# mdejong/MetalBT709Decoder

Measured on AMD Instinct MI355X. Metric: Gpixel/s, 4k NV12->sRGB BGRA decode (output pixels), higher is better.
Workload: dtype f32

## Files before the change

include/bt709hip_ext.h:

```cpp
#ifndef BT709HIP_EXT_H
#define BT709HIP_EXT_H

#include "bt709hip.h"

#ifdef __cplusplus
extern "C" {
#endif

typedef struct bt709hip_pool bt709hip_pool;

typedef struct {
  int32_t device_ordinal;
  int32_t compute_units;
  int32_t wavefront_size;
  int32_t lds_bytes_per_block;
  int32_t memory_clock_khz;
  int32_t memory_bus_width_bits;
  int32_t l2_bytes;
  int32_t clock_khz;
  uint64_t total_memory_bytes;
  char name[128];
  char arch[64];
  char pci_bus_id[32];
  char uuid[40];
// ... 4 lines not shown
  BT709HIP_CTX_OPT_GRID_MULT = 1,
  BT709HIP_CTX_OPT_ENCODE_ROW_PAIRS = 2,
  BT709HIP_CTX_OPT_ENCODE_THREADS = 3,
  BT709HIP_CTX_OPT_XCD_BANDS = 4,
  BT709HIP_CTX_OPT_STREAMING_TRIES = 5
} bt709hip_context_option;
int bt709hip_context_set_option(bt709hip_context *ctx, int option, int value);

int bt709hip_stream_create_with_priority(bt709hip_context *ctx, int priority, void **stream);

int bt709hip_event_create(bt709hip_context *ctx, void **event);
int bt709hip_event_destroy(bt709hip_context *ctx, void *event);
int bt709hip_event_record(bt709hip_context *ctx, void *event, void *stream);
int bt709hip_event_synchronize(bt709hip_context *ctx, void *event);
int bt709hip_stream_wait_event(bt709hip_context *ctx, void *stream, void *event);
int bt709hip_event_elapsed_ms(bt709hip_context *ctx, void *start, void *stop, float *ms);

int bt709hip_graph_begin_capture(bt709hip_context *ctx, void *stream);
int bt709hip_graph_end_capture(bt709hip_context *ctx, void *stream, void **graph);
int bt709hip_graph_launch(bt709hip_context *ctx, void *graph, void *stream);
int bt709hip_graph_destroy(bt709hip_context *ctx, void *graph);

int bt709hip_mem_info(bt709hip_context *ctx, size_t *free_bytes, size_t *total_bytes);
int bt709hip_host_alloc(bt709hip_context *ctx, size_t bytes, void **hptr);
int bt709hip_host_free(bt709hip_context *ctx, void *hptr);

typedef enum {
  BT709HIP_OPT_NONTEMPORAL = 1,
  BT709HIP_OPT_HALF_KERNEL = 2,
  BT709HIP_OPT_HALF_WORKGROUPS = 3,
  BT709HIP_OPT_HALF_LDS_KB = 4,
  BT709HIP_OPT_XCD_BANDS = 5,
  BT709HIP_OPT_COALESCE = 6,
  BT709HIP_OPT_COALESCE_MAX_AGE_US = 7
} bt709hip_decoder_option;
int bt709hip_decoder_set_option(bt709hip_decoder *dec, int option, int value);
int bt709hip_decoder_get_option(const bt709hip_decoder *dec, int option, int *value);

int bt709hip_decoder_flush(bt709hip_decoder *dec, void *stream );
int bt709hip_decoder_flush_all(bt709hip_decoder *dec);

int bt709hip_unconvert_batch(bt709hip_decoder *dec, int count, const void *const *ycbcr_words, size_t in_stride, int width, int height,
                             const bt709hip_surface *outs, void *stream, int wait_until_completed);
int bt709hip_decode_half_batch(bt709hip_decoder *dec, int count, const bt709hip_frame *frames, const bt709hip_frame *alphas,
                               const bt709hip_surface *outs, void *stream, int wait_until_completed);
int bt709hip_decode_scaled_batch(bt709hip_decoder *dec, int count, const bt709hip_frame *frames, const bt709hip_frame *alphas,
                                 const bt709hip_surface *outs, void *stream, int wait_until_completed);
int bt709hip_render_scaled_batch(bt709hip_context *ctx, int count, const bt709hip_surface *ins, const bt709hip_surface *outs,
                                 void *stream, int wait_until_completed);
int bt709hip_encode_batch(bt709hip_context *ctx, int count, const bt709hip_surface *ins, const bt709hip_frame *outs, int input_gamma,
                          int output_gamma, void *stream, int wait_until_completed);
int bt709hip_render_scaled_prepare(bt709hip_context *ctx);
int bt709hip_decoder_prepare_format(bt709hip_decoder *dec, int format);
int bt709hip_encoder_prepare(bt709hip_context *ctx, int input_gamma, int output_gamma);

int bt709hip_pool_create(bt709hip_decoder *dec, int width, int height, int depth, bt709hip_pool **out);
int bt709hip_pool_destroy(bt709hip_pool *pool);
int bt709hip_pool_acquire(bt709hip_pool *pool, int *slot, void **y, size_t *y_stride, void **cbcr,
                          size_t *cbcr_stride);
int bt709hip_pool_alpha_plane(bt709hip_pool *pool, int slot, void **alpha, size_t *alpha_stride);
int bt709hip_pool_submit(bt709hip_pool *pool, int slot);
int bt709hip_pool_wait(bt709hip_pool *pool, int slot, const void **bgra, size_t *stride);
int bt709hip_pool_release(bt709hip_pool *pool, int slot);

typedef struct bt709hip_ring bt709hip_ring;
typedef struct {
  int32_t tries;
  int32_t in_candidates;
  int32_t out_candidates;
  int32_t chosen_in, chosen_out;
// ... 89 lines not shown
```

metalbt709decoder_amd/_capi.py:

```python
import ctypes as C
import os

from . import build as _build

c_void_pp = C.POINTER(C.c_void_p)


class Frame(C.Structure):
    _fields_ = [("y", C.c_void_p), ("y_stride", C.c_size_t),
                ("cbcr", C.c_void_p), ("cbcr_stride", C.c_size_t),
                ("width", C.c_int32), ("height", C.c_int32),
                ("matrix", C.c_int32), ("transfer", C.c_int32)]


class Surface(C.Structure):
    _fields_ = [("bgra", C.c_void_p), ("stride", C.c_size_t),
                ("width", C.c_int32), ("height", C.c_int32),
                ("format", C.c_int32), ("reserved", C.c_int32)]


ABI_VERSION = 503

FORMAT_BGRA8_SRGB = 0
FORMAT_RGBA16F = 1

OPT_NONTEMPORAL = 1
OPT_HALF_KERNEL = 2
OPT_HALF_WORKGROUPS = 3
OPT_HALF_LDS_KB = 4
OPT_XCD_BANDS = 5
OPT_COALESCE = 6
OPT_COALESCE_MAX_AGE_US = 7
CTX_OPT_GRID_MULT = 1
CTX_OPT_ENCODE_ROW_PAIRS = 2
CTX_OPT_ENCODE_THREADS = 3
CTX_OPT_XCD_BANDS = 4
CTX_OPT_STREAMING_TRIES = 5


class RingPlacement(C.Structure):
    _fields_ = [("tries", C.c_int32), ("in_candidates", C.c_int32), ("out_candidates", C.c_int32),
                ("chosen_in", C.c_int32), ("chosen_out", C.c_int32), ("probes", C.c_int32),
                ("first_GBps", C.c_float), ("chosen_GBps", C.c_float), ("best_GBps", C.c_float), ("worst_GBps", C.c_float),
                ("out_prescan_GBps", C.c_float * 18), ("out_kept", C.c_int32 * 18),
                ("hunt_ms", C.c_float), ("stopped_by", C.c_int32), ("peak_bytes", C.c_uint64), ("budget_bytes", C.c_uint64),
                ("evicted", C.c_int32), ("reserved", C.c_int32)]


class RingOptions(C.Structure):
    _fields_ = [("max_bytes", C.c_uint64), ("max_ms", C.c_uint32), ("frugal", C.c_int32), ("format", C.c_int32), ("reserved", C.c_int32)]


class LaunchInfo(C.Structure):
    _fields_ = [("grid", C.c_uint32 * 3), ("block", C.c_uint32 * 3), ("launches", C.c_int32), ("xcd_bands", C.c_int32)]


class ScaledLaunchInfo(C.Structure):
    _fields_ = [("grid", C.c_uint32 * 3), ("block", C.c_uint32 * 3), ("taps", C.c_uint32), ("rows", C.c_uint32),
                ("persistent", C.c_uint32), ("balanced", C.c_uint32), ("resident", C.c_uint32), ("reserved", C.c_uint32),
                ("items", C.c_uint64)]


SCALED_TAPS_BYTES, SCALED_TAPS_PAIRS, SCALED_TAPS_WIDE, SCALED_TAPS_SHARED, SCALED_TAPS_ONCE = range(5)


# ... 189 lines not shown
```

metalbt709decoder_amd/csrc/bt709_ring.cpp:

```cpp
#include "../../include/bt709hip_ext.h"

#include <algorithm>
#include <chrono>
#include <cstring>
#include <map>
#include <new>
#include <utility>
#include <vector>

struct bt709hip_ring {
  bt709hip_decoder *dec = nullptr;
  bt709hip_context *ctx = nullptr;
  int width = 0, height = 0, frames = 0, half = 0, has_alpha = 0, format = BT709HIP_FORMAT_BGRA8_SRGB;
  size_t y_bytes = 0, c_bytes = 0, in_stride = 0, out_stride = 0;
  void *d_in = nullptr, *d_out = nullptr;
  std::vector<bt709hip_frame> f, a;
  std::vector<bt709hip_surface> o;
  bt709hip_ring_placement placement;
};

namespace {

constexpr size_t kHuntMinBytes = 256u << 20;
constexpr size_t kReserveBytes = 4ull << 30;
// ... 190 lines not shown
  auto time_left = [&]() { return max_s == 0.0 || now_s() - t_start < max_s; };
  pl.tries = tries;
  pl.budget_bytes = led.budget;

  std::vector<Slab> ins, outs;
  {
    int n_in = frugal ? std::min(tries, BT709_HUNT_FRUGAL_INPUTS) : tries;
    while (n_in > 1 && ((!frugal && static_cast<size_t>(n_in) * in_bytes > led.budget / 4) || static_cast<size_t>(n_in) * in_bytes + 2 * out_bytes > led.budget)) --n_in;
    for (int i = 0; i < n_in; ++i) {
      if (i > 0 && !led.fits(in_bytes + out_bytes)) break;
      void *p = led.take(in_bytes);
      if (p == nullptr) break;
      ins.push_back(Slab{p, 0.0f, true});
    }
  }
  auto free_everything = [&]() {
    for (Slab &s : ins)
      if (s.alive) led.give(s.p, in_bytes), s.alive = false;
    for (Slab &s : outs)
      if (s.alive) led.give(s.p, out_bytes), s.alive = false;
  };
  if (!ins.empty()) {
    void *p = led.take(out_bytes);
    if (p != nullptr) outs.push_back(Slab{p, 0.0f, true});
  }
  if (ins.empty() || outs.empty()) {
    free_everything();
    delete r;
    return BT709HIP_ERR_HIP;
  }

  int bi = 0, bo = 0;
  Prober pr{r};
  int coalesce = 0;
  (void)bt709hip_decoder_get_option(dec, BT709HIP_OPT_COALESCE, &coalesce);
  if (tries > 1 && bt709hip_event_create(ctx, &pr.e0) == BT709HIP_OK && bt709hip_event_create(ctx, &pr.e1) == BT709HIP_OK) {
    if (coalesce > 1) (void)bt709hip_decoder_set_option(dec, BT709HIP_OPT_COALESCE, 0);
    const double px_per_launch = static_cast<double>(width) * height * frames;
    pr.bytes_per_launch = (static_cast<double>(r->y_bytes + r->c_bytes + (r->has_alpha ? r->y_bytes : 0)) + static_cast<double>(ow) * oh * static_cast<double>(out_px_bytes)) * frames;
    const int reps = std::max(3, static_cast<int>((8.0 * 256 * 3840 * 2160 + px_per_launch - 1) / px_per_launch));
    auto alive_outs = [&]() { return static_cast<int>(std::count_if(outs.begin(), outs.end(), [](const Slab &s) { return s.alive; })); };
    auto evict_slowest_out = [&]() {
      int worst = -1;
      for (size_t k = 0; k < outs.size(); ++k)
        if (outs[k].alive && (worst < 0 || outs[k].rate < outs[static_cast<size_t>(worst)].rate)) worst = static_cast<int>(k);
      if (worst < 0 || alive_outs() <= 1) return false;
      led.give(outs[static_cast<size_t>(worst)].p, out_bytes);
      outs[static_cast<size_t>(worst)].alive = false;
      ++led.evicted;
      return true;
    };
    outs[0].rate = pr.measure(ins[0].p, outs[0].p, reps, 0.15);
    int target = tries;
    while (pr.rc == BT709HIP_OK) {
      bool stuck = false;
      while (static_cast<int>(outs.size()) < target && pr.rc == BT709HIP_OK) {
        if (!time_left()) {
          pl.stopped_by = 2;
          stuck = true;
          break;
        }
        while (!led.fits(out_bytes) && evict_slowest_out()) pl.stopped_by = pl.stopped_by ? pl.stopped_by : 1;
        void *p = led.fits(out_bytes) ? led.take(out_bytes) : nullptr;
        if (p == nullptr) {
          pl.stopped_by = pl.stopped_by ? pl.stopped_by : 1;
          stuck = true;
          break;
        }
        outs.push_back(Slab{p, 0.0f, true});
        outs.back().rate = pr.measure(ins[0].p, p, reps, BT709_HUNT_WARM_S);
// ... 23 lines not shown
          break;
        }
        probed[{static_cast<int>(i), o}] = i == 0 ? outs[static_cast<size_t>(o)].rate : pr.measure(ins[i].p, outs[static_cast<size_t>(o)].p, reps, BT709_HUNT_WARM_S);
      }
    pl.probes = static_cast<int>(probed.size());
    if (pr.rc == BT709HIP_OK && !probed.empty()) {
      pl.first_GBps = outs[0].rate;
      std::vector<std::pair<float, std::pair<int, int>>> ranked;
      for (const auto &kv : probed) ranked.push_back({kv.second, kv.first});
      std::sort(ranked.begin(), ranked.end(), [](const auto &x, const auto &y) { return x.first > y.first; });
      pl.best_GBps = ranked.front().first;
      pl.worst_GBps = ranked.back().first;
      bi = ranked.front().second.first, bo = ranked.front().second.second;
      pl.chosen_GBps = ranked.front().first;
      std::vector<std::pair<int, int>> finalists;
      for (size_t k = 0; k < ranked.size() && k < 3; ++k) finalists.push_back(ranked[k].second);
      const std::pair<int, int> first_pair{0, 0};
      if (std::find(kept.begin(), kept.end(), 0) != kept.end() && std::find(finalists.begin(), finalists.end(), first_pair) == finalists.end())
        finalists.push_back(first_pair);
      float best = -1.0f;
      if (finalists.size() > 1)
        for (const auto &io : finalists) {
          if (pr.rc != BT709HIP_OK) break;
          if (!time_left()) {
            pl.stopped_by = 2;
            break;
          }
          const float v = pr.measure(ins[static_cast<size_t>(io.first)].p, outs[static_cast<size_t>(io.second)].p, BT709_HUNT_CONFIRM_X * reps, BT709_HUNT_WARM_S);
          if (v > best) best = v, bi = io.first, bo = io.second;
        }
      if (best > 0.0f) pl.chosen_GBps = best;
    }
    if (coalesce > 1) (void)bt709hip_decoder_set_option(dec, BT709HIP_OPT_COALESCE, coalesce);
  }
  if (pr.e0) (void)bt709hip_event_destroy(ctx, pr.e0);
  if (pr.e1) (void)bt709hip_event_destroy(ctx, pr.e1);
  pl.in_candidates = static_cast<int>(ins.size());
  if (pl.out_candidates == 0) pl.out_candidates = static_cast<int>(outs.size());
  pl.chosen_in = bi;
  pl.chosen_out = bo;
  pl.evicted = led.evicted;
  void *keep_in = ins[static_cast<size_t>(bi)].alive ? ins[static_cast<size_t>(bi)].p : nullptr;
  void *keep_out = outs[static_cast<size_t>(bo)].alive ? outs[static_cast<size_t>(bo)].p : nullptr;
  ins[static_cast<size_t>(bi)].alive = false;
  outs[static_cast<size_t>(bo)].alive = false;
  pl.peak_bytes = led.peak;
  free_everything();
  if (pl.tries > 1) pl.hunt_ms = static_cast<float>((now_s() - t_start) * 1e3);
  if (pr.rc != BT709HIP_OK || keep_in == nullptr || keep_out == nullptr) {
    if (keep_in) (void)bt709hip_free(ctx, keep_in);
    if (keep_out) (void)bt709hip_free(ctx, keep_out);
    const int rc = pr.rc != BT709HIP_OK ? pr.rc : BT709HIP_ERR_HIP;
    delete r;
    return rc;
  }
  bind_slabs(r, keep_in, keep_out);
  *out = r;
  return BT709HIP_OK;
}

int bt709hip_ring_frames(const bt709hip_ring *r) { return r ? r->frames : BT709HIP_ERR_INVALID_ARG; }

int bt709hip_ring_frame(const bt709hip_ring *r, int index, bt709hip_frame *frame, bt709hip_frame *alpha, bt709hip_surface *out) {
  if (r == nullptr || index < 0 || index >= r->frames) return BT709HIP_ERR_INVALID_ARG;
  if (frame) *frame = r->f[static_cast<size_t>(index)];
  if (alpha) {
// ... 98 lines not shown
```

metalbt709decoder_amd/csrc/shim_coalesce.cpp:

```cpp
#include "shim_internal.h"

namespace bt709shim __attribute__((visibility("hidden"))) {

int issue_queue(bt709hip_decoder *dec, PendingQueue &q) {
  if (q.frames.empty()) return BT709HIP_OK;
  std::vector<bt709hip_frame> frames, alphas;
  std::vector<bt709hip_surface> outs;
  frames.swap(q.frames);
  alphas.swap(q.alphas);
  outs.swap(q.outs);
  return decode_batch_now(dec, static_cast<int>(frames.size()), frames.data(), q.with_alphas ? alphas.data() : nullptr, outs.data(),
                          q.stream, 0);
}

namespace {
int64_t now_us() {
  return std::chrono::duration_cast<std::chrono::microseconds>(std::chrono::steady_clock::now().time_since_epoch()).count();
}
}

int flush_decoder(bt709hip_decoder *dec, hipStream_t s, bool all, bool aged_only) {
  std::lock_guard<std::mutex> lock(dec->queue_mutex);
  int rc = BT709HIP_OK;
  const int64_t limit = aged_only ? now_us() - dec->coalesce_max_age_us : 0;
  for (PendingQueue &q : dec->queues) {
    if (q.frames.empty()) continue;
    const bool aged = dec->coalesce_max_age_us > 0 && q.oldest_us <= limit;
    if (aged_only ? (aged || q.stream == s) : (all || q.stream == s))
      if (int e = issue_queue(dec, q)) rc = rc ? rc : e;
  }
  return rc;
}

int flush_stream(bt709hip_context *ctx, hipStream_t s, const bt709hip_decoder *skip) {
  if (ctx == nullptr || ctx->n_coalescing.load(std::memory_order_acquire) == 0) return BT709HIP_OK;
  const bool aged_too = !capturing(s);
  std::lock_guard<std::mutex> lock(ctx->coalescing_mutex);
  int rc = BT709HIP_OK;
  for (bt709hip_decoder *d : ctx->coalescing)
    if (d != skip)
      if (int e = flush_decoder(d, s, false, aged_too)) rc = rc ? rc : e;
  return rc;
}

int set_coalescing(bt709hip_decoder *dec, int n) {
  bt709hip_context *ctx = dec->ctx;
  const bool now = n > 1;
  if (now && ctx != nullptr) {
    std::lock_guard<std::mutex> lock(ctx->coalescing_mutex);
    if (std::find(ctx->coalescing.begin(), ctx->coalescing.end(), dec) == ctx->coalescing.end()) ctx->coalescing.push_back(dec);
    ctx->n_coalescing.store(static_cast<int>(ctx->coalescing.size()), std::memory_order_release);
  }
  int rc = BT709HIP_OK;
  {
    std::lock_guard<std::mutex> lock(dec->queue_mutex);
    if (!now)
      for (PendingQueue &q : dec->queues)
        if (int e = issue_queue(dec, q)) rc = rc ? rc : e;
    dec->coalesce.store(now ? n : 0);
  }
  if (!now && ctx != nullptr) {
    std::lock_guard<std::mutex> lock(ctx->coalescing_mutex);
    auto it = std::find(ctx->coalescing.begin(), ctx->coalescing.end(), dec);
    if (it != ctx->coalescing.end()) ctx->coalescing.erase(it);
    ctx->n_coalescing.store(static_cast<int>(ctx->coalescing.size()), std::memory_order_release);
  }
  return rc;
}
// ... 26 lines not shown
    if (q != nullptr)
      if (int rc = issue_queue(dec, *q)) return rc;
    return decode_batch_now(dec, count, frames, alphas, outs, stream, wait_until_completed);
  }
  {
    DecodeParams p;
    BatchInfo info;
    if (int rc = gather_batch(dec, count, frames, alphas, outs, OutShape::kSame, stream, &p, &info)) return rc;
    if (p.width == 0) return BT709HIP_OK;
  }
  if (q == nullptr) {
    dec->queues.emplace_back();
    q = &dec->queues.back();
    q->stream = s;
  }
  if (!q->frames.empty()) {
    const bool fits = q->frames.size() + static_cast<size_t>(count) <= static_cast<size_t>(n) &&
                      same_shape(q->frames[0], frames[0]) && q->frames[0].transfer == frames[0].transfer &&
                      q->outs[0].stride == outs[0].stride && q->outs[0].format == outs[0].format &&
                      q->with_alphas == (alphas != nullptr) && (alphas == nullptr || q->alphas[0].y_stride == alphas[0].y_stride);
    if (!fits)
      if (int rc = issue_queue(dec, *q)) return rc;
  }
  q->with_alphas = alphas != nullptr;
  if (q->frames.empty()) q->oldest_us = now_us();
  q->frames.insert(q->frames.end(), frames, frames + count);
  if (alphas != nullptr) q->alphas.insert(q->alphas.end(), alphas, alphas + count);
  q->outs.insert(q->outs.end(), outs, outs + count);
  set_kernel_name("(queued: coalescing submit)");
  if (q->frames.size() >= static_cast<size_t>(n)) return issue_queue(dec, *q);
  return BT709HIP_OK;
}

}

extern "C" {

int bt709hip_decoder_flush(bt709hip_decoder *dec, void *stream) {
  if (dec == nullptr) return BT709HIP_ERR_INVALID_ARG;
  if (dec->ctx == nullptr) return BT709HIP_OK;
  if (int rc = bind(dec->ctx)) return rc;
  return flush_decoder(dec, pick(dec->ctx, stream), false);
}

int bt709hip_decoder_flush_all(bt709hip_decoder *dec) {
  if (dec == nullptr) return BT709HIP_ERR_INVALID_ARG;
  if (dec->ctx == nullptr) return BT709HIP_OK;
  if (int rc = bind(dec->ctx)) return rc;
  return flush_decoder(dec, nullptr, true);
}

}
```

metalbt709decoder_amd/csrc/shim_core.cpp:

```cpp
#include "shim_internal.h"

namespace bt709shim __attribute__((visibility("hidden"))) {

namespace {
thread_local hipError_t tl_hip_error = hipSuccess;
thread_local const char *tl_kernel_name = "";
thread_local bt709::ScaledLaunchRecord tl_scaled_launch = {};
thread_local bool tl_scaled_launched = false;
}

void set_kernel_name(const char *name) { tl_kernel_name = name; }
const char *kernel_name() { return tl_kernel_name; }
hipError_t last_hip_error() { return tl_hip_error; }
const bt709::ScaledLaunchRecord *scaled_launch() { return tl_scaled_launched ? &tl_scaled_launch : nullptr; }
static void store_scaled_launch(const bt709::ScaledLaunchRecord &record) { tl_scaled_launch = record, tl_scaled_launched = true; }

int hip_fail(hipError_t e) {
  tl_hip_error = e;
  (void)hipGetLastError();
  return BT709HIP_ERR_HIP;
}

int bind(const bt709hip_context *ctx) {
  if (ctx == nullptr) return BT709HIP_ERR_INVALID_ARG;
// ... 68 lines not shown
  *out = ctx;
  return BT709HIP_OK;
}

int bt709hip_abi_version(void) { return BT709HIP_VERSION; }

int bt709hip_context_set_option(bt709hip_context *ctx, int option, int value) {
  if (ctx == nullptr) return BT709HIP_ERR_INVALID_ARG;
  switch (option) {
    case BT709HIP_CTX_OPT_GRID_MULT:
      ctx->grid_mult = value <= 0 ? 2 : clamp_int(value, 1, 64);
      ctx->grid_blocks = ctx->props.multiProcessorCount * 8 * ctx->grid_mult;
      return BT709HIP_OK;
    case BT709HIP_CTX_OPT_ENCODE_ROW_PAIRS:
      ctx->encode_row_pairs = clamp_int(value, 0, 64);
      return BT709HIP_OK;
    case BT709HIP_CTX_OPT_ENCODE_THREADS:
      ctx->encode_threads = clamp_int(value, 0, 1024) / 64 * 64;
      return BT709HIP_OK;
    case BT709HIP_CTX_OPT_XCD_BANDS:
      ctx->xcd_bands = value != 0;
      return BT709HIP_OK;
    case BT709HIP_CTX_OPT_STREAMING_TRIES:
      ctx->streaming_tries = value <= 0 ? 4 : clamp_int(value, 1, 32);
      return BT709HIP_OK;
    default:
      return BT709HIP_ERR_INVALID_ARG;
  }
}

int bt709hip_context_destroy(bt709hip_context *ctx) {
  if (ctx == nullptr) return BT709HIP_OK;
  if (hipSetDevice(ctx->device) == hipSuccess && ctx->default_stream) {
    (void)hipStreamSynchronize(ctx->default_stream);
    (void)hipStreamDestroy(ctx->default_stream);
    for (auto &row : ctx->encoders)
      for (EncoderTables &t : row) {
        if (t.d_per_byte) (void)hipFree(t.d_per_byte);
        if (t.d_from_linear) (void)hipFree(t.d_from_linear);
      }
    if (ctx->d_render_encode) (void)hipFree(ctx->d_render_encode);
    if (ctx->d_render_lin) (void)hipFree(ctx->d_render_lin);
  }
  delete ctx;
  return BT709HIP_OK;
}

int bt709hip_context_info(const bt709hip_context *ctx, bt709hip_device_info *info) {
  if (ctx == nullptr || info == nullptr) return BT709HIP_ERR_INVALID_ARG;
  std::memset(info, 0, sizeof *info);
  info->device_ordinal = ctx->device;
  info->compute_units = ctx->props.multiProcessorCount;
  info->wavefront_size = ctx->props.warpSize;
  info->lds_bytes_per_block = static_cast<int32_t>(ctx->props.sharedMemPerBlock);
  info->memory_clock_khz = ctx->props.memoryClockRate;
  info->memory_bus_width_bits = ctx->props.memoryBusWidth;
  info->l2_bytes = ctx->props.l2CacheSize;
  info->clock_khz = ctx->props.clockRate;
  info->total_memory_bytes = ctx->props.totalGlobalMem;
  std::snprintf(info->name, sizeof info->name, "%s", ctx->props.name);
  std::snprintf(info->arch, sizeof info->arch, "%s", ctx->props.gcnArchName);
  if (hipDeviceGetPCIBusId(info->pci_bus_id, static_cast<int>(sizeof info->pci_bus_id), ctx->device) != hipSuccess) {
    (void)hipGetLastError();
    std::snprintf(info->pci_bus_id, sizeof info->pci_bus_id, "%04x:%02x:%02x.0", ctx->props.pciDomainID, ctx->props.pciBusID, ctx->props.pciDeviceID);
  }
  hipUUID uuid;
// ... 256 lines not shown
```

metalbt709decoder_amd/csrc/shim_decode.cpp:

```cpp
#include "shim_internal.h"

namespace bt709shim __attribute__((visibility("hidden"))) {

int required_transfer(int gamma) {
  switch (gamma) {
    case BT709HIP_GAMMA_SRGB: return BT709HIP_TRANSFER_SRGB;
    case BT709HIP_GAMMA_LINEAR: return BT709HIP_TRANSFER_LINEAR;
    default: return BT709HIP_TRANSFER_ITU_R_709_2;
  }
}

int validate(const bt709hip_decoder *dec, const bt709hip_frame *f, const bt709hip_frame *a,
             const bt709hip_surface *o, int out_w, int out_h, int render_w, int render_h) {
  if (f == nullptr || o == nullptr) return BT709HIP_ERR_INVALID_ARG;
  if (f->width < 0 || f->height < 0) return BT709HIP_ERR_INVALID_ARG;
  if (o->width != out_w || o->height != out_h) return BT709HIP_ERR_SIZE_MISMATCH;
  if (render_w != out_w || render_h != out_h) return BT709HIP_ERR_SIZE_MISMATCH;
  if (a != nullptr && (a->width != f->width || a->height != f->height)) return BT709HIP_ERR_SIZE_MISMATCH;
  if (f->matrix != BT709HIP_MATRIX_ITU_R_709_2) return BT709HIP_ERR_MATRIX;
  if (f->transfer != required_transfer(dec->gamma)) return BT709HIP_ERR_TRANSFER;
  if (a != nullptr && a->transfer != BT709HIP_TRANSFER_LINEAR) return BT709HIP_ERR_ALPHA_TRANSFER;
  if ((f->width & 1) || (f->height & 1)) return BT709HIP_ERR_ODD_DIMENSIONS;
  if (dec->has_alpha && a == nullptr) return BT709HIP_ERR_INVALID_ARG;
  if (f->width == 0 || f->height == 0) return BT709HIP_OK;
// ... 136 lines not shown
  const int n = dec->coalesce;
  (void)set_coalescing(dec, 0);
  dec->ctx = ctx;
  (void)set_coalescing(dec, n);
  return BT709HIP_OK;
}

int bt709hip_decoder_set_alpha_fill(bt709hip_decoder *dec, int alpha_byte) {
  if (dec == nullptr || alpha_byte < 0 || alpha_byte > 255) return BT709HIP_ERR_INVALID_ARG;
  if (int rc = bt709hip_decoder_flush_all(dec)) return rc;
  dec->alpha_fill = static_cast<uint32_t>(alpha_byte);
  return BT709HIP_OK;
}

int bt709hip_decoder_get_gamma(const bt709hip_decoder *dec) {
  return dec ? dec->gamma : BT709HIP_ERR_INVALID_ARG;
}

int bt709hip_decoder_has_alpha(const bt709hip_decoder *dec) { return dec ? dec->has_alpha : BT709HIP_ERR_INVALID_ARG; }

bt709hip_context *bt709hip_decoder_context(const bt709hip_decoder *dec) { return dec ? dec->ctx : nullptr; }

int bt709hip_decoder_set_option(bt709hip_decoder *dec, int option, int value) {
  if (dec == nullptr) return BT709HIP_ERR_INVALID_ARG;
  if (int rc = bt709hip_decoder_flush_all(dec)) return rc;
  switch (option) {
    case BT709HIP_OPT_NONTEMPORAL: dec->nontemporal = value != 0; return BT709HIP_OK;
    case BT709HIP_OPT_HALF_KERNEL: dec->half_rep = clamp_int(value, -1, 1); return BT709HIP_OK;
    case BT709HIP_OPT_HALF_WORKGROUPS: dec->half_workgroups = clamp_int(value, 0, 1 << 20); return BT709HIP_OK;
    case BT709HIP_OPT_HALF_LDS_KB: dec->half_lds_kb = clamp_int(value, 0, 160); return BT709HIP_OK;
    case BT709HIP_OPT_XCD_BANDS: dec->xcd_bands = clamp_int(value, 0, 2); return BT709HIP_OK;
    case BT709HIP_OPT_COALESCE: return set_coalescing(dec, value <= 1 ? 0 : clamp_int(value, 2, kMaxBatch));
    case BT709HIP_OPT_COALESCE_MAX_AGE_US: dec->coalesce_max_age_us = value < 0 ? 0 : value; return BT709HIP_OK;
    default: return BT709HIP_ERR_INVALID_ARG;
  }
}

int bt709hip_decoder_get_option(const bt709hip_decoder *dec, int option, int *value) {
  if (dec == nullptr || value == nullptr) return BT709HIP_ERR_INVALID_ARG;
  switch (option) {
    case BT709HIP_OPT_NONTEMPORAL: *value = dec->nontemporal ? 1 : 0; return BT709HIP_OK;
    case BT709HIP_OPT_HALF_KERNEL: *value = dec->half_rep; return BT709HIP_OK;
    case BT709HIP_OPT_HALF_WORKGROUPS: *value = dec->half_workgroups; return BT709HIP_OK;
    case BT709HIP_OPT_HALF_LDS_KB: *value = dec->half_lds_kb; return BT709HIP_OK;
    case BT709HIP_OPT_XCD_BANDS: *value = dec->xcd_bands; return BT709HIP_OK;
    case BT709HIP_OPT_COALESCE: *value = dec->coalesce; return BT709HIP_OK;
    case BT709HIP_OPT_COALESCE_MAX_AGE_US: *value = dec->coalesce_max_age_us; return BT709HIP_OK;
    default: return BT709HIP_ERR_INVALID_ARG;
  }
}

int bt709hip_decoder_setup(bt709hip_decoder *dec) {
  if (dec == nullptr) return BT709HIP_ERR_INVALID_ARG;
  std::lock_guard<std::mutex> lock(dec->setup_mutex);
  if (dec->ctx == nullptr) return BT709HIP_ERR_NOT_SETUP;
  if (dec->ready) return BT709HIP_OK;
  if (int rc = bind(dec->ctx)) return rc;

  TransferTable t;
  TransferTable enc;
  UniformTable enc_u;
  if (!build_transfer_table(dec->gamma, &t) || !build_transfer_table(kGammaLinear, &enc) || enc.buckets_log.empty() ||
      !build_uniform_table(kGammaLinear, 256, &enc_u))
    return BT709HIP_ERR_UNSUPPORTED;
  dec->table_n = t.n;
  const bool log_form = !t.buckets_log.empty();
  const std::vector<TransferBucket> &unit = log_form ? t.buckets_log : t.buckets_unit;
  const float uniform_magic = 8388608.0f / static_cast<float>(t.n);
  uint32_t uniform_first;
  std::memcpy(&uniform_first, &uniform_magic, sizeof uniform_first);
  dec->unit1_magic = log_form ? t.log_add : uniform_magic;
  dec->unit1_first = log_form ? t.log_first : uniform_first;
  dec->unit1_shift = log_form ? 16u : 0u;
  dec->table_unit_bytes = static_cast<uint32_t>(unit.size() * sizeof(TransferBucket));
  dec->table_linear_bytes = static_cast<uint32_t>(t.buckets_linear.size() * sizeof(TransferBucketLinear));
  dec->encode_log_add = enc.log_add;
  dec->encode_log_first = enc.log_first;
  dec->encode_bytes = static_cast<uint32_t>(enc.buckets_log.size() * sizeof(TransferBucket));
  void *d_unit = nullptr, *d_linear = nullptr, *d_enc = nullptr, *d_enc_u = nullptr;
  const uint32_t enc_u_bytes = static_cast<uint32_t>(enc_u.buckets.size() * sizeof(TransferBucket));
// ... 68 lines not shown
  fold_align(&info->in_align, f0.cbcr_stride);
  if (planes_a) fold_align(&info->in_align, alphas[0].y_stride);
  fold_align(&info->out_align, o0.stride);
  if (shape != OutShape::kAny && (f0.height / 2 > kMaxGridYZ || o0.height > 2 * kMaxGridYZ)) return BT709HIP_ERR_UNSUPPORTED;
  if (f0.width == 0 || f0.height == 0 || o0.width == 0 || o0.height == 0) return BT709HIP_OK;

  if (info->uniform && count > 1) {
    p->uniform = 1;
    p->step_y = byte_step(frames[0].y, frames[1].y);
    p->step_cbcr = byte_step(frames[0].cbcr, frames[1].cbcr);
    p->step_alpha = planes_a ? byte_step(alphas[0].y, alphas[1].y) : 0;
    p->step_out = byte_step(outs[0].bgra, outs[1].bgra);
  }
  set_tables(p, dec);
  p->width = static_cast<uint32_t>(f0.width);
  p->height = static_cast<uint32_t>(f0.height);
  p->y_stride = static_cast<uint32_t>(f0.y_stride);
  p->cbcr_stride = static_cast<uint32_t>(f0.cbcr_stride);
  p->alpha_stride = planes_a ? static_cast<uint32_t>(alphas[0].y_stride) : 0;
  p->out_stride = static_cast<uint32_t>(o0.stride);
  p->out_width = static_cast<uint32_t>(o0.width);
  p->out_height = static_cast<uint32_t>(o0.height);
  p->alpha_word = dec->alpha_fill << 24;
  return BT709HIP_OK;
}

}
}

}

namespace bt709shim __attribute__((visibility("hidden"))) {

int decode_batch_now(bt709hip_decoder *dec, int count, const bt709hip_frame *frames, const bt709hip_frame *alphas,
                     const bt709hip_surface *outs, void *stream, int wait_until_completed) {
  DecodeParams p;
  BatchInfo info;
  if (int rc = gather_batch(dec, count, frames, alphas, outs, OutShape::kSame, stream, &p, &info)) return rc;
  if (p.width == 0) return BT709HIP_OK;
  hipStream_t s = pick(dec->ctx, stream);
  if (info.format == BT709HIP_FORMAT_RGBA16F) {
    if (int rc = ensure_half_table(dec, stream)) return rc;
    last_launch_shape() = LaunchShape{};
    set_kernel_name(launch_decode_rgba16f(p, dec->half, count, dec->has_alpha != 0, info.in_align, info.out_align,
                                           static_cast<uint32_t>(dec->ctx->props.multiProcessorCount), dec->xcd_bands != 0, s));
    return finish_launch(s, wait_until_completed);
  }
  const bool fast = (p.width % 4) == 0 && info.in_align >= 4 && info.out_align >= 16;
  const uint32_t gx = fast ? quads_tiles(p.width) : grid_x_for(dec->ctx, p.height / 2, count);
  const uint32_t threads = quads_block_threads(p.width);
  last_launch_shape() = LaunchShape{};
  set_kernel_name(launch_decode(p, count, fast ? kVariantQuads : kVariantBlocks, dec->has_alpha != 0,
                                 dec->gamma == kGammaSRGB, dec->nontemporal, dec->xcd_bands, gx, threads, s));
  return finish_launch(s, wait_until_completed);
}

}

extern "C" {

int bt709hip_decode_batch(bt709hip_decoder *dec, int count, const bt709hip_frame *frames,
                          const bt709hip_frame *alphas, const bt709hip_surface *outs, void *stream,
                          int wait_until_completed) {
  if (dec != nullptr && dec->coalesce > 1) return coalescing_submit(dec, count, frames, alphas, outs, stream, wait_until_completed);
  if (dec != nullptr && dec->ctx != nullptr && dec->ctx->n_coalescing.load(std::memory_order_acquire) != 0) {
    if (int rc = bind(dec->ctx)) return rc;
    FLUSH_STREAM(dec->ctx, stream);
  }
  return decode_batch_now(dec, count, frames, alphas, outs, stream, wait_until_completed);
}

int bt709hip_decode(bt709hip_decoder *dec, const bt709hip_frame *frame, const bt709hip_frame *alpha,
                    const bt709hip_surface *out, int render_width, int render_height, void *stream,
                    int wait_until_completed) {
  if (dec == nullptr) return BT709HIP_ERR_INVALID_ARG;
  if (int rc = ensure_setup(dec, stream)) return rc;
  if (int rc = validate(dec, frame, alpha, out, frame ? frame->width : 0, frame ? frame->height : 0, render_width,
                        render_height))
    return rc;
  return bt709hip_decode_batch(dec, 1, frame, alpha, out, stream, wait_until_completed);
}

int bt709hip_decode_half_batch(bt709hip_decoder *dec, int count, const bt709hip_frame *frames,
                               const bt709hip_frame *alphas, const bt709hip_surface *outs, void *stream,
                               int wait_until_completed) {
  DecodeParams p;
  BatchInfo info;
  if (dec != nullptr) FLUSH_STREAM(dec->ctx, stream);
  if (int rc = gather_batch(dec, count, frames, alphas, outs, OutShape::kHalf, stream, &p, &info)) return rc;
  if (p.width == 0) return BT709HIP_OK;
  hipStream_t s = pick(dec->ctx, stream);
  const bool wide = info.in_align >= 4 && info.out_align >= 8;
  const uint32_t gx = wide ? quads_tiles(p.width) : (p.width / 2 + kBlockThreads - 1) / kBlockThreads;
  const uint32_t threads = wide ? quads_block_threads(p.width) : kBlockThreads;
  const uint32_t cus = static_cast<uint32_t>(dec->ctx->props.multiProcessorCount);
  const uint64_t tile_rows = static_cast<uint64_t>((p.width / 4 + kRepBlockThreads - 1) / kRepBlockThreads) *
                             (p.height / 2) * static_cast<uint32_t>(count);
  const bool rep = wide && dec->half_rep != 0 && (dec->half_rep > 0 || tile_rows >= 8ull * cus);
  const uint32_t rep_groups = dec->half_workgroups > 0 ? static_cast<uint32_t>(dec->half_workgroups) : cus;
  const uint32_t rep_lds = (dec->half_lds_kb > 0 ? static_cast<uint32_t>(dec->half_lds_kb) : 160u) * 1024u;
  const char *name = rep ? launch_decode_half_rep(p, count, dec->has_alpha != 0, dec->nontemporal, rep_groups, rep_lds, s) : nullptr;
  set_kernel_name(name ? name : launch_decode_half(p, count, wide, dec->has_alpha != 0, dec->nontemporal, gx, threads, s));
// ... 45 lines not shown
```

metalbt709decoder_amd/csrc/shim_internal.h:

```cpp
#pragma once
#include "../../include/bt709hip_ext.h"

#include <hip/hip_runtime.h>

#include <algorithm>
#include <atomic>
#include <chrono>
#include <cstdio>
#include <cstdlib>
#include <cstring>
#include <limits>
#include <mutex>
#include <new>
#include <vector>

#include "bt709_constants.h"
#include "bt709_kernels.h"
#include "transfer_tables.h"

using namespace bt709;

struct EncoderTables {
  void *d_per_byte = nullptr;
  void *d_from_linear = nullptr;
  uint32_t from_linear_bytes = 0;
  uint32_t from_linear_n = 0;
  float split = 0.0f, coarse_scale = 1.0f;
  uint32_t coarse_offset = 0;
};

struct bt709hip_context {
  int device = 0;
  hipDeviceProp_t props;
  hipStream_t default_stream = nullptr;
  int grid_mult = 2;
  int grid_blocks = 0;
  int encode_row_pairs = 0, encode_threads = 0;
  int xcd_bands = 1;
  int streaming_tries = 4;
  std::mutex encoder_mutex;
  EncoderTables encoders[3][3];
  void *d_render_encode = nullptr, *d_render_lin = nullptr;
  uint32_t render_encode_bytes = 0, render_encode_log_first = 0;
  float render_encode_log_add = 0.0f;
  std::atomic<int> n_coalescing{0};
  std::mutex coalescing_mutex;
  std::vector<bt709hip_decoder *> coalescing;
};

struct PendingQueue {
  hipStream_t stream = nullptr;
  bool with_alphas = false;
  int64_t oldest_us = 0;
  std::vector<bt709hip_frame> frames, alphas;
  std::vector<bt709hip_surface> outs;
};

struct bt709hip_decoder {
  bt709hip_context *ctx = nullptr;
  int gamma = BT709HIP_GAMMA_APPLE;
  int has_alpha = 0;
  std::atomic<uint32_t> alpha_fill{0xFF};
  std::atomic<bool> nontemporal{true};
  std::atomic<int> half_rep{-1};
  std::atomic<int> half_workgroups{0};
  std::atomic<int> half_lds_kb{0};
  std::atomic<int> xcd_bands{1};
  std::atomic<int> coalesce{0};
  std::atomic<int> coalesce_max_age_us{0};
  std::mutex queue_mutex;
  std::vector<PendingQueue> queues;
  std::mutex setup_mutex;
  std::atomic<bool> ready{false};
  uint32_t table_n = 0;
  float unit1_magic = 0.0f;
  uint32_t unit1_first = 0, unit1_shift = 0;
  void *d_table_unit = nullptr;
  uint32_t table_unit_bytes = 0;
  void *d_table_linear = nullptr;
  uint32_t table_linear_bytes = 0;
  void *d_encode = nullptr;
  uint32_t encode_bytes = 0;
  float encode_log_add = 0.0f;
  uint32_t encode_log_first = 0;
  void *d_encode_u = nullptr;
  uint32_t encode_u_bytes = 0, encode_u_n = 0;
  bool half_ready = false;
  HalfParams half = {};
};

struct bt709hip_pool {
  struct Slot {
    hipStream_t stream = nullptr;
    uint8_t *h_in = nullptr, *h_out = nullptr;
    uint8_t *d_in = nullptr, *d_out = nullptr;
    bool busy = false;
    bool acquired = false;
  };
  bt709hip_decoder *dec = nullptr;
  int width = 0, height = 0;
  size_t in_bytes = 0, out_bytes = 0;
  std::vector<Slot> slots;
// ... 27 lines not shown

constexpr int kMaxGridYZ = 65535;

int upload_table(const void *src, size_t bytes, void **dst);
bool capturing(hipStream_t s);
int finish_launch(hipStream_t s, int wait_until_completed);

int required_transfer(int gamma);
int validate(const bt709hip_decoder *dec, const bt709hip_frame *f, const bt709hip_frame *a, const bt709hip_surface *o, int out_w,
             int out_h, int render_w, int render_h);
int ensure_setup(bt709hip_decoder *dec, void *stream);
int ensure_half_table(bt709hip_decoder *dec, void *stream);
void set_tables(DecodeParams *p, const bt709hip_decoder *dec);
int64_t byte_step(const void *a, const void *b);
bool evenly_spaced(int count, const bt709hip_frame *frames, const bt709hip_frame *alphas, const bt709hip_surface *outs);
uint32_t grid_x_for(const bt709hip_context *ctx, uint32_t rows, int frames);
enum class OutShape { kSame, kHalf, kAny };

struct BatchInfo {
  bool uniform = false;
  uint32_t in_align = 16;
  uint32_t out_align = 16;
  int format = BT709HIP_FORMAT_BGRA8_SRGB;
};
int gather_batch(bt709hip_decoder *dec, int count, const bt709hip_frame *frames, const bt709hip_frame *alphas,
                 const bt709hip_surface *outs, OutShape shape, void *stream, DecodeParams *p, BatchInfo *info);
int decode_batch_now(bt709hip_decoder *dec, int count, const bt709hip_frame *frames, const bt709hip_frame *alphas,
                     const bt709hip_surface *outs, void *stream, int wait_until_completed);

int encoder_tables(bt709hip_context *ctx, int input_gamma, int output_gamma, hipStream_t s);

int issue_queue(bt709hip_decoder *dec, PendingQueue &q);
int flush_decoder(bt709hip_decoder *dec, hipStream_t s, bool all, bool aged_only = false);
int flush_stream(bt709hip_context *ctx, hipStream_t s, const bt709hip_decoder *skip = nullptr);
int set_coalescing(bt709hip_decoder *dec, int n);
int coalescing_submit(bt709hip_decoder *dec, int count, const bt709hip_frame *frames, const bt709hip_frame *alphas,
                      const bt709hip_surface *outs, void *stream, int wait_until_completed);

#define FLUSH_STREAM(ctx, stream)                                                        \
  do {                                                                                   \
    if ((ctx) != nullptr)                                                                \
      if (int _rc = flush_stream((ctx), pick((ctx), (stream)))) return _rc;              \
  } while (0)

}

using namespace bt709shim;
```

metalbt709decoder_amd/csrc/shim_introspect.cpp:

```cpp
#include "shim_internal.h"

extern "C" {


int bt709hip_copy_probe(bt709hip_context *ctx, void *dst, const void *src, size_t bytes, void *stream) {
  if (int rc = bind(ctx)) return rc;
  if (bytes == 0) return BT709HIP_OK;
  if (dst == nullptr || src == nullptr || (bytes & 15) || !aligned(dst, 16) || !aligned(src, 16))
    return BT709HIP_ERR_INVALID_ARG;
  FLUSH_STREAM(ctx, stream);
  set_kernel_name(launch_copy_probe(dst, src, bytes, pick(ctx, stream)));
  HIP_TRY(hipGetLastError());
  return BT709HIP_OK;
}

int bt709hip_malloc_streaming(bt709hip_context *ctx, size_t bytes, int tries, void **dptr, float *rates_GBps, int *chosen) {
  if (dptr == nullptr) return BT709HIP_ERR_INVALID_ARG;
  *dptr = nullptr;
  if (chosen) *chosen = -1;
  if (bytes == 0 || tries < 1 || tries > 32) return BT709HIP_ERR_INVALID_ARG;
  if (rates_GBps)
    for (int i = 0; i < tries; ++i) rates_GBps[i] = 0.0f;
  if (int rc = bind(ctx)) return rc;
  const size_t half = (bytes / 2) & ~static_cast<size_t>(4095);
  hipEvent_t e0 = nullptr, e1 = nullptr;
  hipStream_t s = ctx->default_stream;
  const bool probing = tries > 1 && half >= (1u << 20) && hipEventCreate(&e0) == hipSuccess && hipEventCreate(&e1) == hipSuccess;
  auto probe = [&](void *slab) -> float {
    uint8_t *p = static_cast<uint8_t *>(slab);
    for (int w = 0; w < 2; ++w) {
      launch_copy_probe(p + half, p, half, s);
      (void)hipMemsetAsync(p, 0, bytes, s);
    }
    (void)hipEventRecord(e0, s);
    for (int r = 0; r < 4; ++r) {
      launch_copy_probe(p + half, p, half, s);
      (void)hipMemsetAsync(p, 0, bytes, s);
    }
    (void)hipEventRecord(e1, s);
    float ms = 0.0f;
    if (hipEventSynchronize(e1) != hipSuccess || hipEventElapsedTime(&ms, e0, e1) != hipSuccess || ms <= 0.0f) ms = 1e9f;
    return static_cast<float>(4.0 * (2.0 * static_cast<double>(half) + static_cast<double>(bytes)) / (ms * 1e-3) / 1e9);
  };
  void *best_p = nullptr, *loser = nullptr;
  int best = -1;
  float best_rate = -1.0f;
  for (int i = 0; i < (probing ? tries : 1); ++i) {
    void *p = nullptr;
    hipError_t e = hipMalloc(&p, bytes);
    if (e != hipSuccess && loser != nullptr) {
      (void)hipGetLastError();
      (void)hipFree(loser);
      loser = nullptr;
      e = hipMalloc(&p, bytes);
    }
    if (loser != nullptr) (void)hipFree(loser), loser = nullptr;
// ... 155 lines not shown
```

Baseline: 1164.

## Distribute consecutive default-stream decode calls across side streams

```diff
diff --git a/include/bt709hip_ext.h b/include/bt709hip_ext.h
--- a/include/bt709hip_ext.h
+++ b/include/bt709hip_ext.h
@@ -60,10 +60,12 @@
   BT709HIP_OPT_HALF_LDS_KB = 4,
   BT709HIP_OPT_XCD_BANDS = 5,
   BT709HIP_OPT_COALESCE = 6,
-  BT709HIP_OPT_COALESCE_MAX_AGE_US = 7
+  BT709HIP_OPT_COALESCE_MAX_AGE_US = 7,
+  BT709HIP_OPT_DECODE_LANES = 8
 } bt709hip_decoder_option;
 int bt709hip_decoder_set_option(bt709hip_decoder *dec, int option, int value);
 int bt709hip_decoder_get_option(const bt709hip_decoder *dec, int option, int *value);
+
 
 int bt709hip_decoder_flush(bt709hip_decoder *dec, void *stream );
 int bt709hip_decoder_flush_all(bt709hip_decoder *dec);
diff --git a/metalbt709decoder_amd/_capi.py b/metalbt709decoder_amd/_capi.py
--- a/metalbt709decoder_amd/_capi.py
+++ b/metalbt709decoder_amd/_capi.py
@@ -31,6 +31,7 @@
 OPT_XCD_BANDS = 5
 OPT_COALESCE = 6
 OPT_COALESCE_MAX_AGE_US = 7
+OPT_DECODE_LANES = 8
 CTX_OPT_GRID_MULT = 1
 CTX_OPT_ENCODE_ROW_PAIRS = 2
 CTX_OPT_ENCODE_THREADS = 3
diff --git a/metalbt709decoder_amd/csrc/bt709_ring.cpp b/metalbt709decoder_amd/csrc/bt709_ring.cpp
--- a/metalbt709decoder_amd/csrc/bt709_ring.cpp
+++ b/metalbt709decoder_amd/csrc/bt709_ring.cpp
@@ -246,10 +246,12 @@
 
   int bi = 0, bo = 0;
   Prober pr{r};
-  int coalesce = 0;
+  int coalesce = 0, lanes = -1;
   (void)bt709hip_decoder_get_option(dec, BT709HIP_OPT_COALESCE, &coalesce);
+  (void)bt709hip_decoder_get_option(dec, BT709HIP_OPT_DECODE_LANES, &lanes);
   if (tries > 1 && bt709hip_event_create(ctx, &pr.e0) == BT709HIP_OK && bt709hip_event_create(ctx, &pr.e1) == BT709HIP_OK) {
     if (coalesce > 1) (void)bt709hip_decoder_set_option(dec, BT709HIP_OPT_COALESCE, 0);
+    if (lanes != 0) (void)bt709hip_decoder_set_option(dec, BT709HIP_OPT_DECODE_LANES, 0);
     const double px_per_launch = static_cast<double>(width) * height * frames;
     pr.bytes_per_launch = (static_cast<double>(r->y_bytes + r->c_bytes + (r->has_alpha ? r->y_bytes : 0)) + static_cast<double>(ow) * oh * static_cast<double>(out_px_bytes)) * frames;
     const int reps = std::max(3, static_cast<int>((8.0 * 256 * 3840 * 2160 + px_per_launch - 1) / px_per_launch));
@@ -339,6 +341,7 @@
       if (best > 0.0f) pl.chosen_GBps = best;
     }
     if (coalesce > 1) (void)bt709hip_decoder_set_option(dec, BT709HIP_OPT_COALESCE, coalesce);
+    if (lanes != 0) (void)bt709hip_decoder_set_option(dec, BT709HIP_OPT_DECODE_LANES, lanes);
   }
   if (pr.e0) (void)bt709hip_event_destroy(ctx, pr.e0);
   if (pr.e1) (void)bt709hip_event_destroy(ctx, pr.e1);
diff --git a/metalbt709decoder_amd/csrc/shim_coalesce.cpp b/metalbt709decoder_amd/csrc/shim_coalesce.cpp
--- a/metalbt709decoder_amd/csrc/shim_coalesce.cpp
+++ b/metalbt709decoder_amd/csrc/shim_coalesce.cpp
@@ -9,6 +9,8 @@
   frames.swap(q.frames);
   alphas.swap(q.alphas);
   outs.swap(q.outs);
+  if (dec->ctx != nullptr && q.stream == dec->ctx->default_stream)
+    if (int rc = lanes_join(dec->ctx)) return rc;
   return decode_batch_now(dec, static_cast<int>(frames.size()), frames.data(), q.with_alphas ? alphas.data() : nullptr, outs.data(),
                           q.stream, 0);
 }
@@ -32,8 +34,11 @@
   return rc;
 }
 
-int flush_stream(bt709hip_context *ctx, hipStream_t s, const bt709hip_decoder *skip) {
-  if (ctx == nullptr || ctx->n_coalescing.load(std::memory_order_acquire) == 0) return BT709HIP_OK;
+int flush_stream(bt709hip_context *ctx, hipStream_t s, const bt709hip_decoder *skip, bool join_lanes) {
+  if (ctx == nullptr) return BT709HIP_OK;
+  if (join_lanes && s == ctx->default_stream)
+    if (int rc = lanes_join(ctx)) return rc;
+  if (ctx->n_coalescing.load(std::memory_order_acquire) == 0) return BT709HIP_OK;
   const bool aged_too = !capturing(s);
   std::lock_guard<std::mutex> lock(ctx->coalescing_mutex);
   int rc = BT709HIP_OK;
@@ -126,6 +131,44 @@
   return BT709HIP_OK;
 }
 
+
+int lanes_join_locked(bt709hip_context *ctx) {
+  DecodeLanes &l = ctx->lanes;
+  hipError_t e = hipSuccess;
+  for (int i = 0; i < kLanes - 1; ++i) {
+    if (l.busy[i] && e == hipSuccess) {
+      e = hipEventRecord(l.done[i], l.side[i]);
+      if (e == hipSuccess) e = hipStreamWaitEvent(ctx->default_stream, l.done[i], 0);
+    }
+    l.busy[i] = l.forked[i] = false;
+  }
+  l.fork_recorded = false;
+  for (int &n : l.n_calls) n = 0;
+  l.next = 0;
+  l.active.store(0, std::memory_order_release);
+  return e == hipSuccess ? BT709HIP_OK : hip_fail(e);
+}
+
+int lanes_join_slow(bt709hip_context *ctx) {
+  if (int rc = bind(ctx)) return rc;
+  std::lock_guard<std::mutex> lock(ctx->lanes.mutex);
+  return lanes_join_locked(ctx);
+}
+
+void lanes_destroy(bt709hip_context *ctx) {
+  DecodeLanes &l = ctx->lanes;
+  std::lock_guard<std::mutex> lock(l.mutex);
+  for (int i = 0; i < kLanes - 1; ++i) {
+    if (l.side[i]) (void)hipStreamSynchronize(l.side[i]), (void)hipStreamDestroy(l.side[i]);
+    if (l.done[i]) (void)hipEventDestroy(l.done[i]);
+    l.side[i] = nullptr, l.done[i] = nullptr, l.busy[i] = l.forked[i] = false;
+  }
+  if (l.fork) (void)hipEventDestroy(l.fork);
+  l.fork = nullptr;
+  l.failed = true;
+  l.active.store(0, std::memory_order_release);
+}
+
 }
 
 extern "C" {
diff --git a/metalbt709decoder_amd/csrc/shim_core.cpp b/metalbt709decoder_amd/csrc/shim_core.cpp
--- a/metalbt709decoder_amd/csrc/shim_core.cpp
+++ b/metalbt709decoder_amd/csrc/shim_core.cpp
@@ -124,6 +124,7 @@
 int bt709hip_context_destroy(bt709hip_context *ctx) {
   if (ctx == nullptr) return BT709HIP_OK;
   if (hipSetDevice(ctx->device) == hipSuccess && ctx->default_stream) {
+    lanes_destroy(ctx);
     (void)hipStreamSynchronize(ctx->default_stream);
     (void)hipStreamDestroy(ctx->default_stream);
     for (auto &row : ctx->encoders)
diff --git a/metalbt709decoder_amd/csrc/shim_decode.cpp b/metalbt709decoder_amd/csrc/shim_decode.cpp
--- a/metalbt709decoder_amd/csrc/shim_decode.cpp
+++ b/metalbt709decoder_amd/csrc/shim_decode.cpp
@@ -192,6 +192,7 @@
     case BT709HIP_OPT_XCD_BANDS: dec->xcd_bands = clamp_int(value, 0, 2); return BT709HIP_OK;
     case BT709HIP_OPT_COALESCE: return set_coalescing(dec, value <= 1 ? 0 : clamp_int(value, 2, kMaxBatch));
     case BT709HIP_OPT_COALESCE_MAX_AGE_US: dec->coalesce_max_age_us = value < 0 ? 0 : value; return BT709HIP_OK;
+    case BT709HIP_OPT_DECODE_LANES: dec->decode_lanes = value < 0 ? -1 : (value < 2 ? 0 : clamp_int(value, 2, kLanes)); return BT709HIP_OK;
     default: return BT709HIP_ERR_INVALID_ARG;
   }
 }
@@ -206,6 +207,7 @@
     case BT709HIP_OPT_XCD_BANDS: *value = dec->xcd_bands; return BT709HIP_OK;
     case BT709HIP_OPT_COALESCE: *value = dec->coalesce; return BT709HIP_OK;
     case BT709HIP_OPT_COALESCE_MAX_AGE_US: *value = dec->coalesce_max_age_us; return BT709HIP_OK;
+    case BT709HIP_OPT_DECODE_LANES: *value = dec->decode_lanes; return BT709HIP_OK;
     default: return BT709HIP_ERR_INVALID_ARG;
   }
 }
@@ -340,6 +342,115 @@
 
 namespace bt709shim __attribute__((visibility("hidden"))) {
 
+namespace {
+
+int launch_gathered(bt709hip_decoder *dec, const DecodeParams &p, const BatchInfo &info, int count, void *stream, hipStream_t s,
+                    bool half_resident = false) {
+  if (info.format == BT709HIP_FORMAT_RGBA16F) {
+    if (!half_resident)
+      if (int rc = ensure_half_table(dec, stream)) return rc;
+    last_launch_shape() = LaunchShape{};
+    set_kernel_name(launch_decode_rgba16f(p, dec->half, count, dec->has_alpha != 0, info.in_align, info.out_align,
+                                           static_cast<uint32_t>(dec->ctx->props.multiProcessorCount), dec->xcd_bands != 0, s));
+    return BT709HIP_OK;
+  }
+  const bool fast = (p.width % 4) == 0 && info.in_align >= 4 && info.out_align >= 16;
+  const uint32_t gx = fast ? quads_tiles(p.width) : grid_x_for(dec->ctx, p.height / 2, count);
+  const uint32_t threads = quads_block_threads(p.width);
+  last_launch_shape() = LaunchShape{};
+  set_kernel_name(launch_decode(p, count, fast ? kVariantQuads : kVariantBlocks, dec->has_alpha != 0,
+                                 dec->gamma == kGammaSRGB, dec->nontemporal, dec->xcd_bands, gx, threads, s));
+  return BT709HIP_OK;
+}
+
+
+LaneRange plane_range(const void *base, size_t stride, size_t rows, size_t row_bytes) {
+  const uintptr_t lo = reinterpret_cast<uintptr_t>(base);
+  return LaneRange{lo, lo + (rows - 1) * stride + row_bytes};
+}
+void widen(LaneRange *r, LaneRange x) {
+  if (r->lo == r->hi) *r = x;
+  else r->lo = std::min(r->lo, x.lo), r->hi = std::max(r->hi, x.hi);
+}
+bool overlap(const LaneRange &a, const LaneRange &b) { return a.lo < b.hi && b.lo < a.hi; }
+bool same(const LaneRange &a, const LaneRange &b) { return a.lo == b.lo && a.hi == b.hi; }
+
+LaneCall call_ranges(const DecodeParams &p, int count, const bt709hip_frame *frames, const bt709hip_frame *planes_a,
+                     const bt709hip_surface *outs, size_t px) {
+  LaneCall c;
+  for (int i = 0; i < count; ++i) {
+    widen(&c.read[0], plane_range(frames[i].y, p.y_stride, p.height, p.width));
+    widen(&c.read[1], plane_range(frames[i].cbcr, p.cbcr_stride, p.height / 2, p.width));
+    if (planes_a != nullptr) widen(&c.read[2], plane_range(planes_a[i].y, p.alpha_stride, p.height, p.width));
+    widen(&c.write, plane_range(outs[i].bgra, p.out_stride, p.height, static_cast<size_t>(p.width) * px));
+  }
+  return c;
+}
+
+bool conflicts(const DecodeLanes &l, int m, const LaneCall &c) {
+  for (int k = 0; k < l.n_calls[m]; ++k) {
+    const LaneCall &o = l.calls[m][k];
+    if (overlap(c.write, o.write)) return true;
+    for (int j = 0; j < 3; ++j)
+      if (overlap(c.write, o.read[j]) || overlap(c.read[j], o.write)) return true;
+  }
+  return false;
+}
+
+bool side_lane(DecodeLanes &l, int i) {
+  if (l.failed) return false;
+  if (l.side[i] != nullptr) return true;
+  hipError_t e = l.fork != nullptr ? hipSuccess : hipEventCreateWithFlags(&l.fork, hipEventDisableTiming);
+  if (e == hipSuccess) e = hipEventCreateWithFlags(&l.done[i], hipEventDisableTiming);
+  if (e == hipSuccess) e = hipStreamCreateWithFlags(&l.side[i], hipStreamNonBlocking);
+  if (e == hipSuccess) return true;
+  (void)hipGetLastError();
+  if (l.done[i]) (void)hipEventDestroy(l.done[i]);
+  l.done[i] = nullptr, l.side[i] = nullptr;
+  l.failed = true;
+  return false;
+}
+
+bool deal(bt709hip_decoder *dec, const DecodeParams &p, const BatchInfo &info, int count, const LaneCall &c, int n, int *rc) {
+  bt709hip_context *ctx = dec->ctx;
+  DecodeLanes &l = ctx->lanes;
+  std::lock_guard<std::mutex> lock(l.mutex);
+  for (int i = 0; i < n - 1; ++i)
+    if (!side_lane(l, i)) return false;
+  const int turn = l.next < n ? l.next : 0;
+  int lane = turn, hits = 0;
+  for (int m = 0; m < kLanes; ++m)
+    if (m != turn && conflicts(l, m, c)) ++hits, lane = m;
+  bool known = false;
+  for (int k = 0; k < l.n_calls[lane] && !known; ++k) {
+    const LaneCall &o = l.calls[lane][k];
+    known = same(o.write, c.write) && same(o.read[0], c.read[0]) && same(o.read[1], c.read[1]) && same(o.read[2], c.read[2]);
+  }
+  if (hits > 1 || (!known && l.n_calls[lane] == kLaneCalls)) {
+    if ((*rc = lanes_join_locked(ctx)) != BT709HIP_OK) return true;
+    lane = 0, known = false;
+  }
+  hipStream_t s = lane == 0 ? ctx->default_stream : l.side[lane - 1];
+  if (lane > 0 && !l.forked[lane - 1]) {
+    hipError_t e = l.fork_recorded ? hipSuccess : hipEventRecord(l.fork, ctx->default_stream);
+    if (e == hipSuccess) e = hipStreamWaitEvent(s, l.fork, 0);
+    if (e != hipSuccess) {
+      *rc = hip_fail(e);
+      return true;
+    }
+    l.fork_recorded = l.forked[lane - 1] = true;
+  }
+  if (!known) l.calls[lane][l.n_calls[lane]++] = c;
+  if (lane > 0) l.busy[lane - 1] = true;
+  l.next = (turn + 1) % n;
+  l.active.store(1, std::memory_order_release);
+  *rc = launch_gathered(dec, p, info, count, nullptr, s, true);
+  if (*rc == BT709HIP_OK) *rc = finish_launch(s, 0);
+  return true;
+}
+
+}
+
 int decode_batch_now(bt709hip_decoder *dec, int count, const bt709hip_frame *frames, const bt709hip_frame *alphas,
                      const bt709hip_surface *outs, void *stream, int wait_until_completed) {
   DecodeParams p;
@@ -347,20 +458,39 @@
   if (int rc = gather_batch(dec, count, frames, alphas, outs, OutShape::kSame, stream, &p, &info)) return rc;
   if (p.width == 0) return BT709HIP_OK;
   hipStream_t s = pick(dec->ctx, stream);
-  if (info.format == BT709HIP_FORMAT_RGBA16F) {
-    if (int rc = ensure_half_table(dec, stream)) return rc;
-    last_launch_shape() = LaunchShape{};
-    set_kernel_name(launch_decode_rgba16f(p, dec->half, count, dec->has_alpha != 0, info.in_align, info.out_align,
-                                           static_cast<uint32_t>(dec->ctx->props.multiProcessorCount), dec->xcd_bands != 0, s));
-    return finish_launch(s, wait_until_completed);
-  }
-  const bool fast = (p.width % 4) == 0 && info.in_align >= 4 && info.out_align >= 16;
-  const uint32_t gx = fast ? quads_tiles(p.width) : grid_x_for(dec->ctx, p.height / 2, count);
-  const uint32_t threads = quads_block_threads(p.width);
-  last_launch_shape() = LaunchShape{};
-  set_kernel_name(launch_decode(p, count, fast ? kVariantQuads : kVariantBlocks, dec->has_alpha != 0,
-                                 dec->gamma == kGammaSRGB, dec->nontemporal, dec->xcd_bands, gx, threads, s));
+  if (int rc = launch_gathered(dec, p, info, count, stream, s)) return rc;
   return finish_launch(s, wait_until_completed);
+}
+
+static int decode_batch_lanes(bt709hip_decoder *dec, int count, const bt709hip_frame *frames, const bt709hip_frame *alphas,
+                              const bt709hip_surface *outs, void *stream, int wait_until_completed) {
+  bt709hip_context *ctx = dec != nullptr ? dec->ctx : nullptr;
+  if (ctx == nullptr) return decode_batch_now(dec, count, frames, alphas, outs, stream, wait_until_completed);
+  const bool own = stream == nullptr;
+  const bool prev_own = ctx->lanes.prev_own.exchange(own ? 1 : 0, std::memory_order_relaxed) != 0;
+  const int mode = dec->decode_lanes.load(std::memory_order_relaxed);
+  if (!own || !prev_own || mode == 0 || wait_until_completed != 0 || !dec->ready.load(std::memory_order_acquire)) {
+    if (own)
+      if (int rc = lanes_join(ctx)) return rc;
+    return decode_batch_now(dec, count, frames, alphas, outs, stream, wait_until_completed);
+  }
+  DecodeParams p;
+  BatchInfo info;
+  if (int rc = gather_batch(dec, count, frames, alphas, outs, OutShape::kSame, stream, &p, &info)) return rc;
+  if (p.width == 0) return BT709HIP_OK;
+  const bt709hip_frame *planes_a = dec->has_alpha ? alphas : nullptr;
+  const size_t px = info.format == BT709HIP_FORMAT_RGBA16F ? 8 : 4;
+  const uint64_t bytes = static_cast<uint64_t>(p.width) * p.height * static_cast<uint64_t>(count) * (2 * px + 3 + (planes_a ? 2 : 0)) / 2;
+  int n = mode > 0 ? mode : (bytes > kLaneMaxBytes ? 0 : (bytes < kLaneThreeBelow ? 3 : 2));
+  if (n != 0 && info.format == BT709HIP_FORMAT_RGBA16F) {
+    std::lock_guard<std::mutex> lock(dec->setup_mutex);
+    if (!dec->half_ready) n = 0;
+  }
+  int rc = BT709HIP_OK;
+  if (n != 0 && deal(dec, p, info, count, call_ranges(p, count, frames, planes_a, outs, px), n, &rc)) return rc;
+  if ((rc = lanes_join(ctx)) != BT709HIP_OK) return rc;
+  if ((rc = launch_gathered(dec, p, info, count, stream, ctx->default_stream)) != BT709HIP_OK) return rc;
+  return finish_launch(ctx->default_stream, 0);
 }
 
 }
@@ -370,12 +500,15 @@
 int bt709hip_decode_batch(bt709hip_decoder *dec, int count, const bt709hip_frame *frames,
                           const bt709hip_frame *alphas, const bt709hip_surface *outs, void *stream,
                           int wait_until_completed) {
-  if (dec != nullptr && dec->coalesce > 1) return coalescing_submit(dec, count, frames, alphas, outs, stream, wait_until_completed);
+  if (dec != nullptr && dec->coalesce > 1) {
+    if (dec->ctx != nullptr) dec->ctx->lanes.prev_own.store(stream == nullptr ? 1 : 0, std::memory_order_relaxed);
+    return coalescing_submit(dec, count, frames, alphas, outs, stream, wait_until_completed);
+  }
   if (dec != nullptr && dec->ctx != nullptr && dec->ctx->n_coalescing.load(std::memory_order_acquire) != 0) {
     if (int rc = bind(dec->ctx)) return rc;
-    FLUSH_STREAM(dec->ctx, stream);
-  }
-  return decode_batch_now(dec, count, frames, alphas, outs, stream, wait_until_completed);
+    if (int rc = flush_stream(dec->ctx, pick(dec->ctx, stream), nullptr, false)) return rc;
+  }
+  return decode_batch_lanes(dec, count, frames, alphas, outs, stream, wait_until_completed);
 }
 
 int bt709hip_decode(bt709hip_decoder *dec, const bt709hip_frame *frame, const bt709hip_frame *alpha,
diff --git a/metalbt709decoder_amd/csrc/shim_internal.h b/metalbt709decoder_amd/csrc/shim_internal.h
--- a/metalbt709decoder_amd/csrc/shim_internal.h
+++ b/metalbt709decoder_amd/csrc/shim_internal.h
@@ -27,6 +27,32 @@
   uint32_t from_linear_n = 0;
   float split = 0.0f, coarse_scale = 1.0f;
   uint32_t coarse_offset = 0;
+};
+
+constexpr int kLanes = 3;
+constexpr int kLaneCalls = 16;
+constexpr uint64_t kLaneMaxBytes = 364953600ull;
+constexpr uint64_t kLaneThreeBelow = 91238400ull;
+
+struct LaneRange {
+  uintptr_t lo = 0, hi = 0;
+};
+struct LaneCall {
+  LaneRange read[3], write;
+};
+
+struct DecodeLanes {
+  std::atomic<int> active{0};
+  std::atomic<int> prev_own{1};
+  std::mutex mutex;
+  bool failed = false;
+  hipStream_t side[kLanes - 1] = {};
+  hipEvent_t done[kLanes - 1] = {}, fork = nullptr;
+  bool busy[kLanes - 1] = {}, forked[kLanes - 1] = {};
+  bool fork_recorded = false;
+  int next = 0;
+  int n_calls[kLanes] = {};
+  LaneCall calls[kLanes][kLaneCalls];
 };
 
 struct bt709hip_context {
@@ -46,6 +72,7 @@
   std::atomic<int> n_coalescing{0};
   std::mutex coalescing_mutex;
   std::vector<bt709hip_decoder *> coalescing;
+  DecodeLanes lanes;
 };
 
 struct PendingQueue {
@@ -68,6 +95,7 @@
   std::atomic<int> xcd_bands{1};
   std::atomic<int> coalesce{0};
   std::atomic<int> coalesce_max_age_us{0};
+  std::atomic<int> decode_lanes{-1};
   std::mutex queue_mutex;
   std::vector<PendingQueue> queues;
   std::mutex setup_mutex;
@@ -161,10 +189,17 @@
 
 int issue_queue(bt709hip_decoder *dec, PendingQueue &q);
 int flush_decoder(bt709hip_decoder *dec, hipStream_t s, bool all, bool aged_only = false);
-int flush_stream(bt709hip_context *ctx, hipStream_t s, const bt709hip_decoder *skip = nullptr);
+int flush_stream(bt709hip_context *ctx, hipStream_t s, const bt709hip_decoder *skip = nullptr, bool join_lanes = true);
 int set_coalescing(bt709hip_decoder *dec, int n);
 int coalescing_submit(bt709hip_decoder *dec, int count, const bt709hip_frame *frames, const bt709hip_frame *alphas,
                       const bt709hip_surface *outs, void *stream, int wait_until_completed);
+
+int lanes_join_locked(bt709hip_context *ctx);
+int lanes_join_slow(bt709hip_context *ctx);
+inline int lanes_join(bt709hip_context *ctx) {
+  return ctx->lanes.active.load(std::memory_order_acquire) != 0 ? lanes_join_slow(ctx) : BT709HIP_OK;
+}
+void lanes_destroy(bt709hip_context *ctx);
 
 #define FLUSH_STREAM(ctx, stream)                                                        \
   do {                                                                                   \
diff --git a/metalbt709decoder_amd/csrc/shim_introspect.cpp b/metalbt709decoder_amd/csrc/shim_introspect.cpp
--- a/metalbt709decoder_amd/csrc/shim_introspect.cpp
+++ b/metalbt709decoder_amd/csrc/shim_introspect.cpp
@@ -22,6 +22,7 @@
   if (rates_GBps)
     for (int i = 0; i < tries; ++i) rates_GBps[i] = 0.0f;
   if (int rc = bind(ctx)) return rc;
+  if (int rc = lanes_join(ctx)) return rc;
   const size_t half = (bytes / 2) & ~static_cast<size_t>(4095);
   hipEvent_t e0 = nullptr, e1 = nullptr;
   hipStream_t s = ctx->default_stream;
```

Result: no change. 1164 (median of 3 runs) (-0.0%).
